# Spockuto/drand

Hardware: AMD Instinct MI355X
Metric: beacons verified/s (batch chain verify) (higher is better)
Workload: dtype u32 (381-bit Montgomery, 12x32-bit limbs); 1 GPU; configs[1]: 1000000-round chained beacon history per GPU, chain.VerifyBeacon per round; beacons_per_gpu=1000000, segment_len=64, parallelism=range-shard x1

## Files before the change

### drand_amd/_lib.py

```python
from __future__ import annotations

import ctypes
import os

_HERE = os.path.dirname(os.path.abspath(__file__))
LIB_PATH = os.environ.get("DRAND_AMD_LIB", os.path.join(_HERE, "libblsverify.so"))

BLSV_OK = 0
BLSV_EINVAL = -1
BLSV_EHIP = -2
BLSV_ENOGROUP = -3
BLSV_ENOTENOUGH = -4

AGG_OK = 0
AGG_OK_V2 = 1
AGG_V1_RECOVER_FAIL = 2
AGG_V1_INVALID = 3
AGG_V2_RECOVER_FAIL = 4

REJ_OK = 0
REJ_LENGTH = 1
REJ_FLAG = 2
REJ_INF_NONZERO = 3
REJ_X_GE_P = 4
# ... 30 lines not shown
sz = ctypes.c_size_t

SIGNATURES = {
    "blsv_version": (ctypes.c_char_p, []),
    "blsv_device_count": (ctypes.c_int, []),
    "blsv_create": (ctypes.c_int, [ctypes.c_int, ctypes.POINTER(vp)]),
    "blsv_destroy": (None, [vp]),
    "blsv_last_error": (ctypes.c_char_p, [vp]),
    "blsv_synchronize": (ctypes.c_int, [vp]),
    "blsv_set_group": (ctypes.c_int, [vp, u8p, sz, sz]),
    "blsv_verify_chained": (ctypes.c_int, [vp, ctypes.c_uint64, u8p, sz, u8p, sz, u8p, u64p, u8p]),
    "blsv_verify_chained_multi": (ctypes.c_int, [ctypes.POINTER(vp), sz, ctypes.POINTER(sz), ctypes.c_uint64, u8p, sz,
                                                  u8p, sz, u8p, u64p, u8p]),
    "blsv_verify_prevs": (ctypes.c_int, [vp, ctypes.c_uint64, u8p, sz, u8p, sz, u8p, u64p, u8p]),
    "blsv_verify_unchained": (ctypes.c_int, [vp, u64p, ctypes.c_uint64, u8p, sz, u8p, u64p, u8p]),
    "blsv_verify_messages": (ctypes.c_int, [vp, u8p, u8p, u32p, sz, u8p, u8p, u64p, u8p]),
    "blsv_verify_partials": (ctypes.c_int, [vp, u8p, sz, u8p, sz, sz, u8p, u8p]),
    "blsv_verify_partials_multi": (ctypes.c_int, [vp, u8p, u32p, u8p, sz, sz, u8p, u8p]),
    "blsv_recover": (ctypes.c_int, [vp, u8p, sz, u8p, sz, sz, sz, sz, u8p]),
    "blsv_aggregate": (ctypes.c_int, [vp, u8p, sz, u8p, sz, sz, sz, sz, u8p, u8p, u8p, u8p]),
    "blsv_aggregate_round": (ctypes.c_int, [vp, u8p, sz, u8p, sz, u8p, sz, u8p, sz, sz, sz, sz, u8p, u8p, u8p, u8p,
                                             ctypes.POINTER(ctypes.c_int32), u8p]),
    "blsv_sign": (ctypes.c_int, [vp, u8p, ctypes.c_int32, u8p, u32p, sz, u8p]),
    "blsv_verify_chained_dev": (ctypes.c_int, [vp, ctypes.c_uint64, ctypes.c_uint64, ctypes.c_uint64, vp, sz, vp, sz,
                                                vp, vp, vp, vp]),
    "blsv_generate_chained_dev": (ctypes.c_int, [vp, u8p, ctypes.c_uint64, ctypes.c_uint64, vp, sz, vp, sz, vp]),
    "blsv_profile_enable": (ctypes.c_int, [vp, ctypes.c_int]),
    "blsv_profile_read": (ctypes.c_int, [vp, ctypes.POINTER(ctypes.c_double), u64p, u64p, ctypes.c_int]),
    "blsv_lat_trace": (ctypes.c_int, [vp, u64p, ctypes.c_int, ctypes.POINTER(ctypes.c_double), ctypes.c_int]),
    "blsv_test_fp_mul": (ctypes.c_int, [vp, u32p, u32p, sz, u32p]),
    "blsv_test_op": (ctypes.c_int, [vp, ctypes.c_char_p, u32p, sz, u32p]),
    "blsv_test_op_info": (ctypes.c_int, [ctypes.c_int, ctypes.POINTER(ctypes.c_char_p), ctypes.POINTER(ctypes.c_int),
                                         ctypes.POINTER(ctypes.c_int), ctypes.POINTER(ctypes.c_int)]),
    "blsv_test_pairing": (ctypes.c_int, [vp, u32p, u32p, sz, u32p]),
    "blsv_test_hash_to_g2": (ctypes.c_int, [vp, u8p, u32p, sz, u32p, u8p]),
    "blsv_test_final_exp": (ctypes.c_int, [vp, u32p, sz, u32p, u32p]),
    "blsv_test_tail_split": (ctypes.c_int, [vp, sz]),
    "blsv_set_lat_max": (sz, [vp, sz]),
    "blsv_set_chunk": (sz, [vp, sz]),
    "blsv_workspace_bytes": (sz, [vp]),
    "blsv_lat_trace_enable": (ctypes.c_int, [vp, ctypes.c_int]),
    "blsv_test_generic_chains": (ctypes.c_int, [vp, ctypes.c_int]),
    "blsv_test_spec_stats": (ctypes.c_int, [vp, ctypes.POINTER(ctypes.c_uint64), ctypes.POINTER(ctypes.c_uint64)]),
    "blsv_test_lagrange": (ctypes.c_int, [ctypes.POINTER(ctypes.c_uint32), ctypes.c_size_t, ctypes.POINTER(ctypes.c_uint32)]),
    "blsv_service_create": (ctypes.c_int, [ctypes.c_int, ctypes.c_uint32, ctypes.c_uint32, ctypes.POINTER(vp)]),
    "blsv_service_destroy": (None, [vp]),
    "blsv_service_verify_partial": (ctypes.c_int, [vp, u8p, sz, sz, u8p, sz, u8p, sz, u8p, u8p]),
    "blsv_service_verify_recovered": (ctypes.c_int, [vp, u8p, u8p, sz, u8p, u8p, u8p]),
    "blsv_service_stats": (ctypes.c_int, [vp, u64p, u64p, u64p]),
    "blsv_test_service_limits": (ctypes.c_int, [vp, sz, sz, sz, u64p]),
    "blsv_verify_chained_rlc": (ctypes.c_int, [vp, ctypes.c_uint64, u8p, sz, u8p, sz, u8p, u64p, u8p]),
    "blsv_verify_unchained_rlc": (ctypes.c_int, [vp, u64p, ctypes.c_uint64, u8p, sz, u8p, u64p, u8p]),
    "blsv_verify_chained_rlc_dev": (ctypes.c_int, [vp, ctypes.c_uint64, ctypes.c_uint64, ctypes.c_uint64, vp, sz, vp,
                                                    sz, vp, vp, vp, vp]),
    "blsv_set_rlc_group": (sz, [vp, sz]),
    "blsv_rlc_stats": (ctypes.c_int, [vp, u64p, u64p, u64p]),
    "blsv_test_rlc_seed": (ctypes.c_int, [vp, u8p]),
    "blsv_test_rlc_sums": (ctypes.c_int, [vp, ctypes.c_uint64, u8p, sz, u8p, sz, u8p, u8p]),
    "blsv_tlock_open": (ctypes.c_int, [vp, u8p, u8p, sz, u8p, u8p, u8p, u8p]),
    "blsv_tlock_open_dev": (ctypes.c_int, [vp, u8p, vp, sz, vp, vp, vp]),
    "blsv_tlock_stats": (ctypes.c_int, [vp, u64p, u64p]),
    "blsv_tlock_open_rounds": (ctypes.c_int, [vp, u8p, u64p, sz, u8p, sz, u8p, u8p, u8p, u8p]),
    "blsv_tlock_open_rounds_dev": (ctypes.c_int, [vp, u8p, u64p, sz, vp, sz, vp, vp, vp, vp]),
    "blsv_tlock_open_rounds_stats": (ctypes.c_int, [vp, u64p, u64p]),
    "blsv_set_tlock_dense_min": (sz, [vp, sz]),
    "blsv_set_tlock_lat_max": (sz, [vp, sz]),
# ... 73 lines not shown
```

### drand_amd/csrc/fp.h

```cpp
#pragma once
#include <stdint.h>
#include "bls_constants.h"

#ifdef BLS_HOST
#include <stddef.h>
#define DI inline
#define NOINL static inline
namespace bls {
extern unsigned long long g_fp_mul_count;
}
#define BLS_COUNT_MUL() (++::bls::g_fp_mul_count)
#else
#include <hip/hip_runtime.h>
#define DI __device__ __forceinline__
#define NOINL static __device__ __noinline__
#define BLS_COUNT_MUL() ((void)0)
#endif

namespace bls {

struct fp {
  uint32_t l[12];
};

DI fp fp_load_const(const uint32_t (&c)[12]) {
  fp r;
#pragma unroll
  for (int i = 0; i < 12; i++) r.l[i] = c[i];
  return r;
}

DI fp fp_zero() {
  fp r;
#pragma unroll
  for (int i = 0; i < 12; i++) r.l[i] = 0;
  return r;
}

DI fp fp_one() { return fp_load_const(FP_ONE); }

DI bool fp_raw_is_zero(const fp& a) {
  uint32_t acc = 0;
#pragma unroll
  for (int i = 0; i < 12; i++) acc |= a.l[i];
  return acc == 0;
}

DI bool fp_is_zero(const fp& a) {
  uint32_t z = 0, q = 0;
// ... 220 lines not shown
DI u12 fp_add_raw_u12(const u12& a, const u12& b) {
  u12 r;
  unsigned c = 0;
#pragma unroll
  for (int i = 0; i < 12; i++) r[i] = __builtin_addc(a[i], b[i], c, &c);
  return r;
}

typedef uint32_t u24 __attribute__((ext_vector_type(24)));

template <bool DOT>
DI void fp_mont_dot_t(const uint32_t (&x0)[14], const uint32_t (&y0)[14], const uint32_t (&x1)[14],
                      const uint32_t (&y1)[14], uint32_t (&t)[14]) {
  uint32_t m[14];
  uint64_t c = 0;
#pragma unroll
  for (int k = 0; k < 27; k++) {
    const int lo = k > 13 ? k - 13 : 0, hi = k < 13 ? k : 13;
#pragma unroll
    for (int j = lo; j <= hi; j++) {
      c += (uint64_t)x0[j] * y0[k - j];
      if (DOT) c += (uint64_t)x1[j] * y1[k - j];
    }
    if (k < 14) {
#pragma unroll
      for (int j = 0; j < k; j++) c += (uint64_t)m[j] * P28[k - j];
      m[k] = ((uint32_t)c * P_INV28) & M28;
      c += (uint64_t)m[k] * P28[0];
    } else {
#pragma unroll
      for (int j = k - 13; j < 14; j++) c += (uint64_t)m[j] * P28[k - j];
      t[k - 14] = (uint32_t)c & M28;
    }
    c >>= 28;
  }
  t[13] = (uint32_t)c;
}
template <int NT>
DI u12 fp_mont_dot3(const uint32_t (&x0)[14], const uint32_t (&y0)[14], const uint32_t (&x1)[14],
                    const uint32_t (&y1)[14], const uint32_t (&x2)[14], const uint32_t (&y2)[14]) {
  uint32_t m[14], t[14];
  uint64_t c = 0;
#pragma unroll
  for (int k = 0; k < 27; k++) {
    const int lo = k > 13 ? k - 13 : 0, hi = k < 13 ? k : 13;
#pragma unroll
    for (int j = lo; j <= hi; j++) {
      c += (uint64_t)x0[j] * y0[k - j];
      c += (uint64_t)x1[j] * y1[k - j];
      if (NT == 3) c += (uint64_t)x2[j] * y2[k - j];
    }
    if (k < 14) {
#pragma unroll
      for (int j = 0; j < k; j++) c += (uint64_t)m[j] * P28[k - j];
      m[k] = ((uint32_t)c * P_INV28) & M28;
      c += (uint64_t)m[k] * P28[0];
    } else {
#pragma unroll
      for (int j = k - 13; j < 14; j++) c += (uint64_t)m[j] * P28[k - j];
      t[k - 14] = (uint32_t)c & M28;
    }
    c >>= 28;
  }
  t[13] = (uint32_t)c;
  return fp_join28(t);
}
// ... 108 lines not shown
  return u24_of(fp_join28(t0), fp_join28(t1));
}

template <bool KARA>
DI u24 fp2_mul_body_t(const u24& a, const u12& b0, const u12& b1) {
  if (KARA) return fp2_mul_body_kara(a, b0, b1);
  uint32_t x0[14], x1[14], y0[14], y1[14], yn[14];
  fp_split28(u24_lo(a), x0);
  fp_split28(u24_hi(a), x1);
  fp_split28(b0, y0);
  fp_split28(b1, y1);
  fp_neg28(y1, yn);
  const u12 c0 = fp_mont_dot<true>(x0, y0, x1, yn);
  BLS_SCHED_FENCE();
  const u12 c1 = fp_mont_dot<true>(x0, y1, x1, y0);
  return u24_of(c0, c1);
}
DI u24 fp2_mul_body(const u24& a, const u12& b0, const u12& b1) { return fp2_mul_body_t<BLS_FP2_KARA>(a, b0, b1); }

DI u24 fp2_sqr_body(const u24& a) {
  uint32_t s0[14], s1[14], x[14], y[14];
  fp_split28(u24_lo(a), s0);
  fp_split28(u24_hi(a), s1);
#pragma unroll
  for (int k = 0; k < 14; k++) {
    x[k] = s0[k] + s1[k];
    y[k] = s0[k] + (NEG28_16P[k] - s1[k]);
  }
  const u12 c0 = fp_mont_dot<false>(x, y, x, y);
  BLS_SCHED_FENCE();
#pragma unroll
  for (int k = 0; k < 14; k++) x[k] = s0[k] << 1;
  const u12 c1 = fp_mont_dot<false>(x, s1, x, s1);
  return u24_of(c0, c1);
}

NOINL u24 fp2_mul_u24(u24 a) {
  BLS_COUNT_MUL();
  BLS_COUNT_MUL();
  BLS_COUNT_MUL();
  const unsigned l = bls_lane();
  u12 b0, b1;
#pragma unroll
  for (int i = 0; i < 12; i++) {
    b0[i] = g_fp2_arg[i * BLS_LANES + l];
    b1[i] = g_fp2_arg[(12 + i) * BLS_LANES + l];
  }
  return fp2_mul_body(a, b0, b1);
}

NOINL u24 fp2_sqr_u24(u24 a) {
  BLS_COUNT_MUL();
  BLS_COUNT_MUL();
  return fp2_sqr_body(a);
}

DI u12 fp_to_u12(const fp& a) {
  u12 v;
#pragma unroll
  for (int i = 0; i < 12; i++) v[i] = a.l[i];
  return v;
}

DI fp fp_from_u12(const u12& v) {
  fp a;
#pragma unroll
// ... 317 lines not shown
```

### drand_amd/csrc/pairing.h

```cpp
#pragma once
#include "curve.h"

namespace bls {

struct g2proj {
  fp2 x, y, z;
};

DI fp2 fp2_mul_3b(const fp2& c) {
  fp2 x4 = fp2_dbl(fp2_dbl(fp2_mul_xi(c)));
  return fp2_add(fp2_dbl(x4), x4);
}

template <bool INL = false>
DI void miller_dbl_step(g2proj& t, fp2& l00, fp2& l01, fp2& l11, const fp& xp, const fp& yp) {
  auto mul = [](const fp2& a, const fp2& b) { return INL ? fp2_mul_inl(a, b) : fp2_mul(a, b); };
  auto sqr = [](const fp2& a) { return INL ? fp2_sqr_inl(a) : fp2_sqr(a); };
  fp2 A = fp2_half(mul(t.x, t.y));
  fp2 B = sqr(t.y);
  fp2 C = sqr(t.z);
  fp2 E = fp2_mul_3b(C);
  fp2 F = fp2_mul3(E);
  fp2 G = fp2_half(fp2_add(B, F));
  fp2 H = fp2_sub(sqr(fp2_add_lazy(t.y, t.z)), fp2_add(B, C));
  fp2 X2 = sqr(t.x);
  l00 = fp2_sub(E, B);
  l01 = fp2_mul_fp(fp2_mul3(X2), xp);
  l11 = fp2_neg(fp2_mul_fp(H, yp));
  t.x = mul(A, fp2_sub(B, F));
  t.y = fp2_sub(sqr(G), fp2_mul3(sqr(E)));
  t.z = mul(B, H);
}



struct g2proj_reg {
  g2proj& t;
  DI fp2 get(int c) const { return c == 0 ? t.x : c == 1 ? t.y : t.z; }
  DI void set(int c, const fp2& v) const {
    if (c == 0) t.x = v;
    else if (c == 1) t.y = v;
    else t.z = v;
  }
};

template <typename TS, typename Put, typename XP, typename YP>
DI void miller_dbl_step_ts(const TS& t, Put put, XP xp, YP yp) {
  const fp2 B = fp2_sqr_inl(t.get(1));
  BLS_SCHED_FENCE();
  const fp2 C = fp2_sqr_inl(t.get(2));
  BLS_SCHED_FENCE();
  const fp2 H = fp2_sub(fp2_sqr_inl(fp2_add_lazy(t.get(1), t.get(2))), fp2_add(B, C));
  BLS_SCHED_FENCE();
  put(2, fp2_neg(fp2_mul_fp_inl(H, yp())));
  BLS_SCHED_FENCE();
  t.set(2, fp2_mul_inl_k<0>(B, H));
  BLS_SCHED_FENCE();
  const fp2 E = fp2_mul_3b(C);
  const fp2 F = fp2_mul3(E);
  const fp2 G = fp2_half(fp2_add(B, F));
  put(0, fp2_sub(E, B));
  const fp2 BF = fp2_sub(B, F);
  const fp2 A = fp2_half(fp2_mul_inl_k<1>(t.get(0), t.get(1)));
  BLS_SCHED_FENCE();
  put(1, fp2_mul_fp_inl(fp2_mul3(fp2_sqr_inl(t.get(0))), xp()));
  BLS_SCHED_FENCE();
  t.set(0, fp2_mul_inl(A, BF));
  BLS_SCHED_FENCE();
  const fp2 G2 = fp2_sqr_inl(G);
  BLS_SCHED_FENCE();
  t.set(1, fp2_sub(G2, fp2_mul3(fp2_sqr_inl(E))));
}

template <typename TS, typename Put, typename Q, typename XP, typename YP>
DI void miller_add_step_ts(const TS& t, Q qload, Put put, XP xp, YP yp) {
  fp2 theta, delta;
  {
    const g2a q = qload();
    theta = fp2_sub(t.get(1), fp2_mul_inl(q.y, t.get(2)));
    BLS_SCHED_FENCE();
    delta = fp2_sub(t.get(0), fp2_mul_inl(q.x, t.get(2)));
    BLS_SCHED_FENCE();
    const fp2 u = fp2_mul_inl(theta, q.x);
    BLS_SCHED_FENCE();
    put(0, fp2_sub(u, fp2_mul_inl(delta, q.y)));
    BLS_SCHED_FENCE();
  }
  put(1, fp2_neg(fp2_mul_fp_inl(theta, xp())));
  BLS_SCHED_FENCE();
  put(2, fp2_mul_fp_inl(delta, yp()));
  BLS_SCHED_FENCE();
  const fp2 C = fp2_sqr_inl(theta);
  BLS_SCHED_FENCE();
  const fp2 D = fp2_sqr_inl(delta);
  BLS_SCHED_FENCE();
  const fp2 E = fp2_mul_inl(D, delta);
  BLS_SCHED_FENCE();
  const fp2 F = fp2_mul_inl(t.get(2), C);
  BLS_SCHED_FENCE();
  const fp2 G = fp2_mul_inl(t.get(0), D);
  BLS_SCHED_FENCE();
  const fp2 H = fp2_sub(fp2_add(E, F), fp2_dbl(G));
  t.set(0, fp2_mul_inl(delta, H));
  BLS_SCHED_FENCE();
// ... 237 lines not shown
```

### drand_amd/csrc/testhooks.cpp

```cpp
#include "../../include/blsverify_testing.h"
#include "host_internal.h"
#include "testops_list.h"

static const bls::TestOpInfo* find_test_op(const char* name, int* op) {
  if (!name) return nullptr;
  const bls::TestOpInfo* tab = bls::test_op_table();
  for (int k = 0; k < bls::TOP_COUNT; k++)
    if (!strcmp(tab[k].name, name)) {
      if (op) *op = k;
      return &tab[k];
    }
  return nullptr;
}

extern "C" {

int blsv_test_lagrange(const uint32_t* idx, size_t t, uint32_t* out) {
  if (!idx || !out) return BLSV_EINVAL;
  for (size_t i = 0; i < t; i++)
    for (size_t j = 0; j < i; j++)
      if (idx[i] == idx[j]) return BLSV_EINVAL;
  host_lagrange(idx, t, out);
  return BLSV_OK;
}

int blsv_test_rlc_seed(blsv_ctx* c, const uint8_t* seed32) {
  if (!c) return BLSV_EINVAL;
  c->rlc.seed_pinned = seed32 != nullptr;
  if (seed32) memcpy(c->rlc.seed, seed32, 32);
  return BLSV_OK;
}

int blsv_test_rlc_sums(blsv_ctx* c, uint64_t first_round, const uint8_t* prev0, size_t prev0_len,
                       const uint8_t* sigs96, size_t n, uint8_t* out_a96, uint8_t* out_b96) {
  if (!c) return BLSV_EINVAL;
  if (!n || !sigs96 || !prev0 || !out_a96 || !out_b96 || (prev0_len != 32 && prev0_len != 96))
    return fail(c, BLSV_EINVAL, "test_rlc_sums: bad arguments");
  (void)hipSetDevice(c->device);
  Tail tail;
  tail.randomized = true;
// ... 120 lines not shown
  if (n > c->cap) return fail(c, BLSV_EINVAL, "test_final_exp: more than the context chunk");
  if (!n) return BLSV_OK;
  DBuf din, dout, dref;
  HIPCHK(c, din.ensure(n * 576));
  HIPCHK(c, dout.ensure(n * 576));
  HIPCHK(c, dref.ensure(n * 576));
  const Staging w = staging(c);
  HIPCHK(c, hipMemcpyAsync(din.p, f, n * 576, hipMemcpyHostToDevice, c->stream));
  HIPCHK(c, hipMemsetAsync(w.cls, 0, n, c->stream));
  blsk::launch_test_pack_fp12(din.as<uint32_t>(), n, w.F, c->stream);
  blsk::launch_test_final_exp_ref(w.F, n, dref.as<uint32_t>(), c->stream);
  const size_t mn = tail_split_main(n, c->tail_q);
  final_exp(c, n, 0, mn, w.cls, c->stream, dout.as<uint32_t>());
  final_exp(c, n, mn, n - mn, w.cls, c->stream, dout.as<uint32_t>());
  blsk::launch_test_unpack_fp12(dout.as<uint32_t>(), n, din.as<uint32_t>(), c->stream);
  HIPCHK(c, hipMemcpyAsync(out_pipeline, din.p, n * 576, hipMemcpyDeviceToHost, c->stream));
  blsk::launch_test_unpack_fp12(dref.as<uint32_t>(), n, dout.as<uint32_t>(), c->stream);
  HIPCHK(c, hipMemcpyAsync(out_ref, dout.p, n * 576, hipMemcpyDeviceToHost, c->stream));
  HIPCHK(c, hipGetLastError());
  HIPCHK(c, hipStreamSynchronize(c->stream));
  return BLSV_OK;
}

int blsv_test_op_info(int index, const char** name, int* in_fp, int* out_fp, int* lanes) {
  if (index < 0 || index >= bls::TOP_COUNT) return BLSV_EINVAL;
  const bls::TestOpInfo& t = bls::test_op_table()[index];
  if (name) *name = t.name;
  if (in_fp) *in_fp = t.nin;
  if (out_fp) *out_fp = t.nout;
  if (lanes) *lanes = t.kind == 3 ? 3 : 1;
  return BLSV_OK;
}

int blsv_test_op(blsv_ctx* c, const char* name, const uint32_t* in, size_t n, uint32_t* out) {
  int op = 0;
  const bls::TestOpInfo* t = find_test_op(name, &op);
  if (!c || !t || (n && (!in || !out))) return BLSV_EINVAL;
  if (n > kMaxChunk) return BLSV_EINVAL;
  if (!n) return BLSV_OK;
  (void)hipSetDevice(c->device);
  const size_t in_bytes = n * (size_t)t->nin * 48, out_bytes = n * (size_t)t->nout * 48;
  DBuf din, dout, dpark;
  HIPCHK(c, din.ensure(in_bytes));
  HIPCHK(c, dout.ensure(out_bytes));
  if (t->kind == 3) HIPCHK(c, dpark.ensure(blsk::TRI_PARK_WORDS(n) * 4));
  HIPCHK(c, hipMemcpyAsync(din.p, in, in_bytes, hipMemcpyHostToDevice, c->stream));
  HIPCHK(c, hipMemsetAsync(dout.p, 0xA5, out_bytes, c->stream));
  const bool ran = t->kind == 2
                       ? blsk::launch_test_op_mf(op, din.as<uint32_t>(), n, dout.as<uint32_t>(), c->stream)
                       : blsk::launch_test_op(op, din.as<uint32_t>(), n, dout.as<uint32_t>(),
                                              t->kind == 3 ? dpark.as<uint32_t>() : nullptr, c->stream);
  if (!ran) return fail(c, BLSV_EINVAL, "test_op: no kernel for this op");
  HIPCHK(c, hipGetLastError());
  HIPCHK(c, hipMemcpyAsync(out, dout.p, out_bytes, hipMemcpyDeviceToHost, c->stream));
  HIPCHK(c, hipStreamSynchronize(c->stream));
  return BLSV_OK;
}

int blsv_test_hash_to_g2(blsv_ctx* c, const uint8_t* msgs, const uint32_t* msg_lens, size_t n, uint32_t* out,
                         uint8_t* inf) {
  if (!c || (n && (!msg_lens || !out || !inf))) return BLSV_EINVAL;
  if (n > kMaxChunk) return BLSV_EINVAL;
  (void)hipSetDevice(c->device);
  int rc = ensure_workspace(c, n);
  if (rc) return rc;
  if (n > c->cap) return fail(c, BLSV_EINVAL, "test_hash_to_g2: more than the context chunk");
// ... 15 lines not shown
```

### drand_amd/csrc/testops.h

```cpp
#pragma once
#include "pairing.h"
#include "tri.h"
#include "testops_list.h"

namespace bls {

DI fp2 t_f2(const fp* x, int k) { return {x[k], x[k + 1]}; }
DI fp6 t_f6(const fp* x, int k) { return {t_f2(x, k), t_f2(x, k + 2), t_f2(x, k + 4)}; }
DI fp12 t_f12(const fp* x, int k) { return {t_f6(x, k), t_f6(x, k + 6)}; }
DI void t_put2(fp* r, int k, const fp2& v) { r[k] = v.c0, r[k + 1] = v.c1; }
DI void t_put6(fp* r, int k, const fp6& v) { t_put2(r, k, v.c0), t_put2(r, k + 2, v.c1), t_put2(r, k + 4, v.c2); }
DI void t_put12(fp* r, int k, const fp12& v) { t_put6(r, k, v.c0), t_put6(r, k + 6, v.c1); }
DI fp t_flag(bool b) {
  fp r = fp_zero();
  r.l[0] = b ? 1u : 0u;
  return r;
}

template <int OP, typename KP16>
DI void test_op_run(const fp* x, fp* r) {
  if constexpr (OP == TOP_fp_mul) r[0] = fp_mul(x[0], x[1]);
  if constexpr (OP == TOP_fp_mul_inl) r[0] = fp_mul_inl(x[0], x[1]);
  if constexpr (OP == TOP_fp_sqr) r[0] = fp_sqr(x[0]);
  if constexpr (OP == TOP_fp_add) r[0] = fp_add(x[0], x[1]);
// ... 28 lines not shown
  if constexpr (OP == TOP_fp2_sqr) t_put2(r, 0, fp2_sqr(t_f2(x, 0)));
  if constexpr (OP == TOP_fp2_sqr_inl) t_put2(r, 0, fp2_sqr_inl(t_f2(x, 0)));
  if constexpr (OP == TOP_fp2_mul_xi) t_put2(r, 0, fp2_mul_xi(t_f2(x, 0)));
  if constexpr (OP == TOP_fp2_neg) t_put2(r, 0, fp2_neg(t_f2(x, 0)));
  if constexpr (OP == TOP_fp2_inv) t_put2(r, 0, fp2_inv(t_f2(x, 0)));
  if constexpr (OP == TOP_fp2_3u_p_2x) t_put2(r, 0, fp2_3u_pm_2x(t_f2(x, 0), t_f2(x, 2), false));
  if constexpr (OP == TOP_fp2_3u_m_2x) t_put2(r, 0, fp2_3u_pm_2x(t_f2(x, 0), t_f2(x, 2), true));
  if constexpr (OP == TOP_kara6_c0) t_put2(r, 0, kara6_c0(t_f2(x, 0), t_f2(x, 2), t_f2(x, 4), t_f2(x, 6), KP16()));
  if constexpr (OP == TOP_kara6_c1) t_put2(r, 0, kara6_c1(t_f2(x, 0), t_f2(x, 2), t_f2(x, 4), t_f2(x, 6), KP16()));
  if constexpr (OP == TOP_kara6_c2) t_put2(r, 0, kara6_c2(t_f2(x, 0), t_f2(x, 2), t_f2(x, 4), t_f2(x, 6), KP16()));
  if constexpr (OP == TOP_fp6_mul_lin) t_put6(r, 0, fp6_mul_lin(t_f6(x, 0), t_f6(x, 6), KP16()));
  if constexpr (OP == TOP_fp6_mul) t_put6(r, 0, fp6_mul(t_f6(x, 0), t_f6(x, 6)));
  if constexpr (OP == TOP_fp6_sqr) t_put6(r, 0, fp6_sqr(t_f6(x, 0)));
  if constexpr (OP == TOP_fp6_mul_by_01) t_put6(r, 0, fp6_mul_by_01(t_f6(x, 0), t_f2(x, 6), t_f2(x, 8)));
  if constexpr (OP == TOP_fp6_mul_by_1) t_put6(r, 0, fp6_mul_by_1(t_f6(x, 0), t_f2(x, 6)));
  if constexpr (OP == TOP_fp6_mul_by_12) t_put6(r, 0, fp6_mul_by_12(t_f6(x, 0), t_f2(x, 6), t_f2(x, 8)));
  if constexpr (OP == TOP_fp6_inv) t_put6(r, 0, fp6_inv(t_f6(x, 0)));
  if constexpr (OP == TOP_fp4_sqr_k7) {
    const fp4 y = fp4_sqr_k7(fp4{t_f2(x, 0), t_f2(x, 2)});
    t_put2(r, 0, y.a), t_put2(r, 2, y.b);
  }
  if constexpr (OP == TOP_fp12_mul) t_put12(r, 0, fp12_mul(t_f12(x, 0), t_f12(x, 12)));
  if constexpr (OP == TOP_fp12_sqr) t_put12(r, 0, fp12_sqr(t_f12(x, 0)));
  if constexpr (OP == TOP_fp12_sqr_lin) t_put12(r, 0, fp12_sqr_lin(t_f12(x, 0), KP16()));
  if constexpr (OP == TOP_fp12_mul_by_014)
    t_put12(r, 0, fp12_mul_by_014(t_f12(x, 0), t_f2(x, 12), t_f2(x, 14), t_f2(x, 16)));
  if constexpr (OP == TOP_line_mul_line)
    t_put12(r, 0, line_mul_line(line{t_f2(x, 0), t_f2(x, 2), t_f2(x, 4)}, line{t_f2(x, 6), t_f2(x, 8), t_f2(x, 10)}));
  if constexpr (OP == TOP_fp12_cyclotomic_sqr) t_put12(r, 0, fp12_cyclotomic_sqr(t_f12(x, 0)));
  if constexpr (OP == TOP_fp12_frob) t_put12(r, 0, fp12_frob(t_f12(x, 0)));
  if constexpr (OP == TOP_fp12_frob2) t_put12(r, 0, fp12_frob2(t_f12(x, 0)));
  if constexpr (OP == TOP_fp12_conj) t_put12(r, 0, fp12_conj(t_f12(x, 0)));
  if constexpr (OP == TOP_fp12_inv) t_put12(r, 0, fp12_inv(t_f12(x, 0)));
}

}
```

### drand_amd/csrc/testops_list.h

```cpp
#pragma once

#define BLS_TEST_OPS(X)                                                                              \
  X(fp_mul, 2, 1, 0) X(fp_mul_inl, 2, 1, 0) X(fp_sqr, 1, 1, 0) X(fp_add, 2, 1, 0) X(fp_sub, 2, 1, 0) \
  X(fp_addsub_add, 2, 1, 0) X(fp_addsub_sub, 2, 1, 0) X(fp_neg, 1, 1, 0) X(fp_half, 1, 1, 0)         \
  X(fp_dbl, 1, 1, 0) X(fp_mul3, 1, 1, 0) X(fp_add_lazy_mul, 3, 2, 0) X(fp_add_lazy2_mul, 5, 2, 0)   \
  X(fp_canon, 1, 1, 0) X(fp_is_zero, 1, 1, 0) X(fp_eq, 2, 1, 0) X(fp_inv_bingcd_raw, 1, 2, 0)        \
  X(fp_inv, 1, 1, 0) X(fp_pow_sqrt_inv, 1, 1, 0)                                                     \
  X(fp2_mul, 4, 2, 0) X(fp2_mul_inl, 4, 2, 0) X(fp2_mul_inl_kara, 4, 2, 0) X(fp2_sqr, 2, 2, 0)       \
  X(fp2_sqr_inl, 2, 2, 0) X(fp2_mul_xi, 2, 2, 0) X(fp2_neg, 2, 2, 0) X(fp2_inv, 2, 2, 0)             \
  X(fp2_3u_p_2x, 4, 2, 0) X(fp2_3u_m_2x, 4, 2, 0) X(fp2_3u_p_2x_lds, 4, 2, 1)                        \
  X(fp2_3u_m_2x_lds, 4, 2, 1) X(kara6_c0, 8, 2, 0) X(kara6_c1, 8, 2, 0) X(kara6_c2, 8, 2, 0)         \
  X(fp6_mul_lin, 12, 6, 0) X(fp6_mul, 12, 6, 0) X(fp6_sqr, 6, 6, 0) X(fp6_mul_by_01, 10, 6, 0)       \
  X(fp6_mul_by_1, 8, 6, 0) X(fp6_mul_by_12, 10, 6, 0) X(fp6_inv, 6, 6, 0) X(fp4_sqr_k7, 4, 4, 0)     \
  X(fp4_sqr_dot, 4, 4, 1) X(fp4_mul, 8, 4, 1) X(fp12_mul, 24, 12, 0) X(fp12_sqr, 12, 12, 0)          \
  X(fp12_sqr_lin, 12, 12, 0) X(fp12_mul_by_014, 18, 12, 0) X(line_mul_line, 12, 12, 0)               \
  X(fp12_cyclotomic_sqr, 12, 12, 0) X(fp12_frob, 12, 12, 0) X(fp12_frob2, 12, 12, 0)                 \
  X(fp12_conj, 12, 12, 0) X(fp12_inv, 12, 12, 0)                                                     \
  X(fp6_mul_lb, 12, 6, 2) X(fp12_mul_by_line_pair_lds, 22, 12, 2)                                    \
  X(tri_cyclotomic_sqr, 12, 12, 3) X(tri_mul_lp, 24, 12, 3) X(tri_sqr_lp, 12, 12, 3)                 \
  X(tri_line_pair, 12, 12, 3) X(tri_frob, 12, 12, 3) X(tri_frob2, 12, 12, 3) X(tri_conj, 12, 12, 3)  \
  X(tri_is_one, 12, 1, 3)

namespace bls {

enum TestOp : int {
#define X(name, nin, nout, kind) TOP_##name,
  BLS_TEST_OPS(X)
#undef X
      TOP_COUNT
};

struct TestOpInfo {
  const char* name;
  int nin, nout, kind;
};
inline const TestOpInfo* test_op_table() {
  static const TestOpInfo tab[TOP_COUNT] = {
#define X(name, nin, nout, kind) {#name, nin, nout, kind},
      BLS_TEST_OPS(X)
#undef X
  };
  return tab;
}

}
```

### drand_amd/csrc/tower.h

```cpp
#pragma once
#include "fp.h"

namespace bls {

struct fp2 {
  fp c0, c1;
};
struct fp6 {
  fp2 c0, c1, c2;
};
struct fp12 {
  fp6 c0, c1;
};

DI fp2 fp2_load_const(const uint32_t (&c)[2][12]) { return {fp_load_const(c[0]), fp_load_const(c[1])}; }
DI fp2 fp2_zero() { return {fp_zero(), fp_zero()}; }
DI fp2 fp2_one() { return {fp_one(), fp_zero()}; }
DI bool fp2_is_zero(const fp2& a) { return fp_is_zero(a.c0) & fp_is_zero(a.c1); }
DI bool fp2_eq(const fp2& a, const fp2& b) { return fp_eq(a.c0, b.c0) & fp_eq(a.c1, b.c1); }
DI fp2 fp2_select(bool c, const fp2& a, const fp2& b) { return {fp_select(c, a.c0, b.c0), fp_select(c, a.c1, b.c1)}; }
DI fp2 fp2_add(const fp2& a, const fp2& b) {
  uint32_t s0[12], d0[12], s1[12], d1[12];
  unsigned c0 = 0, b0 = 0, c1 = 0, b1 = 0;
#pragma unroll
// ... 150 lines not shown
  for (int i = 0; i < 12; i++) {
    r.c0.l[i] = d0[i] & m0;
    r.c1.l[i] = d1[i] & m1;
  }
  return r;
}
DI fp2 fp2_conj(const fp2& a) { return {a.c0, fp_neg(a.c1)}; }

DI u24 fp2_to_u24(const fp2& a) { return u24_of(fp_to_u12(a.c0), fp_to_u12(a.c1)); }
DI fp2 fp2_from_u24(const u24& v) { return {fp_from_u12(u24_lo(v)), fp_from_u12(u24_hi(v))}; }

DI fp2 fp2_mul(const fp2& a, const fp2& b) {
  fp2_arg_store(fp2_to_u24(b));
  return fp2_from_u24(fp2_mul_u24(fp2_to_u24(a)));
}
DI fp2 fp2_sqr(const fp2& a) { return fp2_from_u24(fp2_sqr_u24(fp2_to_u24(a))); }
template <bool KARA>
DI fp2 fp2_mul_inl_t(const fp2& a, const fp2& b) {
  BLS_COUNT_MUL();
  BLS_COUNT_MUL();
  BLS_COUNT_MUL();
  return fp2_from_u24(fp2_mul_body_t<KARA>(fp2_to_u24(a), fp_to_u12(b.c0), fp_to_u12(b.c1)));
}
DI fp2 fp2_mul_inl(const fp2& a, const fp2& b) { return fp2_mul_inl_t<BLS_FP2_KARA_INL>(a, b); }
#ifndef BLS_LINES_KARA
#define BLS_LINES_KARA 3
#endif
template <int SITE>
DI fp2 fp2_mul_inl_k(const fp2& a, const fp2& b) { return fp2_mul_inl_t<((BLS_LINES_KARA >> SITE) & 1) != 0>(a, b); }
DI fp2 fp2_sqr_inl(const fp2& a) {
  BLS_COUNT_MUL();
  BLS_COUNT_MUL();
  return fp2_from_u24(fp2_sqr_body(fp2_to_u24(a)));
}

DI fp2 fp2_mul_fp(const fp2& a, const fp& b) { return {fp_mul(a.c0, b), fp_mul(a.c1, b)}; }
DI fp2 fp2_mul_fp_inl(const fp2& a, const fp& b) {
  const fp c0 = fp_mul_inl(a.c0, b);
  BLS_SCHED_FENCE();
  return {c0, fp_mul_inl(a.c1, b)};
}
DI fp2 fp2_mul3(const fp2& a) { return {fp_mul3(a.c0), fp_mul3(a.c1)}; }

DI fp2 fp2_mul_xi(const fp2& a) {
  uint32_t d[12], e[12], s[12], u[12];
  unsigned bd = 0, ce = 0, cs = 0, bu = 0;
#pragma unroll
  for (int i = 0; i < 12; i++) {
    d[i] = __builtin_subc(a.c0.l[i], a.c1.l[i], bd, &bd);
    s[i] = __builtin_addc(a.c0.l[i], a.c1.l[i], cs, &cs);
    e[i] = __builtin_addc(d[i], P2_RAW[i], ce, &ce);
    u[i] = __builtin_subc(s[i], P2_RAW[i], bu, &bu);
  }
  fp2 r;
#pragma unroll
  for (int i = 0; i < 12; i++) {
    r.c0.l[i] = bd ? e[i] : d[i];
    r.c1.l[i] = bu ? s[i] : u[i];
  }
  return r;
}

DI fp2 fp2_inv(const fp2& a) {
  fp n = fp_add(fp_sqr(a.c0), fp_sqr(a.c1));
  fp ni = fp_inv(n);
  return {fp_mul(a.c0, ni), fp_neg(fp_mul(a.c1, ni))};
// ... 374 lines not shown
```

### drand_amd/engine.py

```python
from __future__ import annotations

import ctypes
from dataclasses import dataclass

from . import _lib
from ._lib import u8p, u32p, u64p


class EngineError(RuntimeError):
    def __init__(self, code, msg):
        super().__init__(f"blsverify error {code}: {msg}")
        self.code = code


@dataclass
class BatchResult:
    ok: list
    first_bad: int | None
    reject_class: list

    @property
    def all_ok(self):
        return self.first_bad is None

# ... 759 lines not shown
                 "final_exp", "pow1_start", "pow1_end", "xmd_done", "sswu_done", "iso_add_done", "cofactor_done",
                 "sig_sqrt_done", "sig_subgroup_done")

    def lat_trace_enable(self, on=True):
        self._check(self.lib.blsv_lat_trace_enable(self._h, 1 if on else 0))

    def lat_trace(self, clear=True):
        n = len(self.LAT_MARKS)
        t = (ctypes.c_uint64 * n)()
        rate = ctypes.c_double()
        got = self.lib.blsv_lat_trace(self._h, t, n, ctypes.byref(rate), 1 if clear else 0)
        if got < 0:
            raise EngineError(got, self.lib.blsv_last_error(self._h).decode())
        t0 = t[0]
        return {k: (t[i] - t0) / rate.value for i, k in enumerate(self.LAT_MARKS[:got]) if t[i] and t0}

    def set_lat_max(self, n):
        return self.lib.blsv_set_lat_max(self._h, int(n))

    def set_chunk(self, items):
        return self.lib.blsv_set_chunk(self._h, int(items))

    def workspace_bytes(self):
        return self.lib.blsv_workspace_bytes(self._h)

    def test_fp_mul(self, a_limbs, b_limbs):
        n = len(a_limbs) // 12
        A = (ctypes.c_uint32 * max(len(a_limbs), 1))(*a_limbs)
        B = (ctypes.c_uint32 * max(len(b_limbs), 1))(*b_limbs)
        O = (ctypes.c_uint32 * max(n * 12, 1))()
        self._check(self.lib.blsv_test_fp_mul(self._h, A, B, n, O))
        return list(O)[:n * 12]

    def test_ops(self):
        ops, k = {}, 0
        name, a, b, c = ctypes.c_char_p(), ctypes.c_int(), ctypes.c_int(), ctypes.c_int()
        while self.lib.blsv_test_op_info(k, ctypes.byref(name), ctypes.byref(a), ctypes.byref(b), ctypes.byref(c)) == 0:
            ops[name.value.decode()] = (a.value, b.value, c.value)
            k += 1
        return ops

    def test_op(self, name, operands):
        if self._ops is None:
            self._ops = self.test_ops()
        nin, nout, _ = self._ops[name]
        if len(operands) % nin:
            raise ValueError(f"{name} takes {nin} Fp elements per item")
        n = len(operands) // nin
        raw = b"".join(int(v).to_bytes(48, "little") for v in operands)
        A = (ctypes.c_uint32 * max(len(raw) // 4, 1)).from_buffer_copy(raw if raw else bytes(4))
        O = (ctypes.c_uint32 * max(n * nout * 12, 1))()
        self._check(self.lib.blsv_test_op(self._h, name.encode(), A, n, O))
        ob = bytes(O)
        return [int.from_bytes(ob[48 * k:48 * k + 48], "little") for k in range(n * nout)]

    def test_pairing(self, p_words, q_words):
        n = len(p_words) // 24
        Pp = (ctypes.c_uint32 * max(len(p_words), 1))(*p_words)
        Q = (ctypes.c_uint32 * max(len(q_words), 1))(*q_words)
        O = (ctypes.c_uint32 * max(n * 144, 1))()
        self._check(self.lib.blsv_test_pairing(self._h, Pp, Q, n, O))
        return list(O)[:n * 144]

    def test_final_exp(self, f_words):
        n = len(f_words) // 144
        Fw = (ctypes.c_uint32 * max(len(f_words), 1))(*f_words)
        A = (ctypes.c_uint32 * max(n * 144, 1))()
        B = (ctypes.c_uint32 * max(n * 144, 1))()
        self._check(self.lib.blsv_test_final_exp(self._h, Fw, n, A, B))
        return list(A)[:n * 144], list(B)[:n * 144]

    def test_tail_split(self, q):
        self._check(self.lib.blsv_test_tail_split(self._h, ctypes.c_size_t(-1).value if q is None else int(q)))

    def test_hash_to_g2(self, msgs):
        n = len(msgs)
        lens = (ctypes.c_uint32 * max(n, 1))(*[len(m) for m in msgs])
# ... 118 lines not shown
```

### include/blsverify_testing.h

```cpp
#ifndef DRAND_AMD_BLSVERIFY_TESTING_H
#define DRAND_AMD_BLSVERIFY_TESTING_H

#include "blsverify.h"

#ifdef __cplusplus
extern "C" {
#endif

int blsv_test_fp_mul(blsv_ctx* ctx, const uint32_t* a, const uint32_t* b, size_t n, uint32_t* out);

int blsv_test_pairing(blsv_ctx* ctx, const uint32_t* p, const uint32_t* q, size_t n, uint32_t* out_f);

int blsv_test_final_exp(blsv_ctx* ctx, const uint32_t* f, size_t n, uint32_t* out_pipeline, uint32_t* out_ref);

int blsv_test_tail_split(blsv_ctx* ctx, size_t q);

int blsv_test_tauth_walk_waves(blsv_ctx* ctx, int waves);

int blsv_test_op(blsv_ctx* ctx, const char* name, const uint32_t* in, size_t n, uint32_t* out);
int blsv_test_op_info(int index, const char** name, int* in_fp, int* out_fp, int* lanes);

int blsv_test_hash_to_g2(blsv_ctx* ctx, const uint8_t* msgs, const uint32_t* msg_lens, size_t n, uint32_t* out,
                         uint8_t* inf);

int blsv_test_generic_chains(blsv_ctx* ctx, int on);

int blsv_test_spec_stats(blsv_ctx* ctx, uint64_t* hits, uint64_t* misses);

int blsv_test_service_limits(blsv_service* svc, size_t chunk, size_t lat_max, size_t arena_entries,
                             uint64_t* sub_launches);

int blsv_profile_enable(blsv_ctx* ctx, int on);
int blsv_lat_trace(blsv_ctx* ctx, uint64_t* ticks, int n, double* ticks_per_us, int clear);
int blsv_lat_trace_enable(blsv_ctx* ctx, int on);
int blsv_profile_read(blsv_ctx* ctx, double* ms, uint64_t* launches, uint64_t* items, int nstages);
int blsv_test_lagrange(const uint32_t* idx, size_t t, uint32_t* out);

int blsv_test_rlc_seed(blsv_ctx* ctx, const uint8_t* seed32);
int blsv_test_rlc_sums(blsv_ctx* ctx, uint64_t first_round, const uint8_t* prev0, size_t prev0_len,
                       const uint8_t* sigs96, size_t n, uint8_t* out_a96, uint8_t* out_b96);

#ifdef __cplusplus
}
#endif

#endif
```

Baseline: 2.512 million beacons/s.

## Fuse G²−E·F in Miller doubling and derive XY from squares

```diff
diff --git a/drand_amd/_lib.py b/drand_amd/_lib.py
--- a/drand_amd/_lib.py
+++ b/drand_amd/_lib.py
@@ -86,6 +86,9 @@
     "blsv_test_op": (ctypes.c_int, [vp, ctypes.c_char_p, u32p, sz, u32p]),
     "blsv_test_op_info": (ctypes.c_int, [ctypes.c_int, ctypes.POINTER(ctypes.c_char_p), ctypes.POINTER(ctypes.c_int),
                                          ctypes.POINTER(ctypes.c_int), ctypes.POINTER(ctypes.c_int)]),
+    "blsv_test_step_op_info": (ctypes.c_int, [ctypes.c_int, ctypes.POINTER(ctypes.c_char_p),
+                                              ctypes.POINTER(ctypes.c_int), ctypes.POINTER(ctypes.c_int),
+                                              ctypes.POINTER(ctypes.c_int)]),
     "blsv_test_pairing": (ctypes.c_int, [vp, u32p, u32p, sz, u32p]),
     "blsv_test_hash_to_g2": (ctypes.c_int, [vp, u8p, u32p, sz, u32p, u8p]),
     "blsv_test_final_exp": (ctypes.c_int, [vp, u32p, sz, u32p, u32p]),
diff --git a/drand_amd/csrc/fp.h b/drand_amd/csrc/fp.h
--- a/drand_amd/csrc/fp.h
+++ b/drand_amd/csrc/fp.h
@@ -10,11 +10,20 @@
 extern unsigned long long g_fp_mul_count;
 }
 #define BLS_COUNT_MUL() (++::bls::g_fp_mul_count)
+#ifdef BLS_HOST_COLUMNS
+namespace bls {
+extern unsigned long long g_col_max;
+}
+#define BLS_COLUMN(c) (::bls::g_col_max = (c) > ::bls::g_col_max ? (c) : ::bls::g_col_max)
+#else
+#define BLS_COLUMN(c) ((void)0)
+#endif
 #else
 #include <hip/hip_runtime.h>
 #define DI __device__ __forceinline__
 #define NOINL static __device__ __noinline__
 #define BLS_COUNT_MUL() ((void)0)
+#define BLS_COLUMN(c) ((void)0)
 #endif
 
 namespace bls {
@@ -301,6 +310,7 @@
       for (int j = k - 13; j < 14; j++) c += (uint64_t)m[j] * P28[k - j];
       t[k - 14] = (uint32_t)c & M28;
     }
+    BLS_COLUMN(c);
     c >>= 28;
   }
   t[13] = (uint32_t)c;
@@ -475,6 +485,36 @@
 #pragma unroll
   for (int k = 0; k < 14; k++) x[k] = s0[k] << 1;
   const u12 c1 = fp_mont_dot<false>(x, s1, x, s1);
+  return u24_of(c0, c1);
+}
+
+DI u24 fp2_sqr_minus_prod_body(const u24& g, const u24& e, const u24& f) {
+  uint32_t g0[14], g1[14], e1[14], f0[14], x0[14], y0[14], x1[14], y1[14];
+  fp_split28(u24_lo(g), g0);
+  fp_split28(u24_hi(g), g1);
+  fp_split28(u24_hi(e), e1);
+  fp_split28(u24_lo(f), f0);
+  {
+    uint32_t e0[14], f1[14];
+    fp_split28(u24_lo(e), e0);
+    fp_split28(u24_hi(f), f1);
+#pragma unroll
+    for (int k = 0; k < 14; k++) {
+      x0[k] = g0[k] + g1[k];
+      y0[k] = g0[k] + (NEG28_16P[k] - g1[k]);
+      x1[k] = f0[k] + f1[k];
+      y1[k] = e1[k] + (NEG28_16P[k] - e0[k]);
+    }
+  }
+  const u12 c0 = fp_mont_dot<true>(x0, y0, x1, y1);
+  BLS_SCHED_FENCE();
+#pragma unroll
+  for (int k = 0; k < 14; k++) {
+    x0[k] = g0[k] << 1;
+    x1[k] = f0[k] << 1;
+    y1[k] = NEG28_16P[k] - e1[k];
+  }
+  const u12 c1 = fp_mont_dot<true>(x0, g1, x1, y1);
   return u24_of(c0, c1);
 }
 
diff --git a/drand_amd/csrc/pairing.h b/drand_amd/csrc/pairing.h
--- a/drand_amd/csrc/pairing.h
+++ b/drand_amd/csrc/pairing.h
@@ -44,6 +44,13 @@
   }
 };
 
+#ifndef BLS_LINES_XY_SQR
+#define BLS_LINES_XY_SQR 1
+#endif
+DI fp2 miller_dbl_xy_open(const fp2& X, const fp2& Y, const fp2& B) {
+  return fp2_sub(fp2_sqr_inl(fp2_add_lazy(X, Y)), B);
+}
+DI fp2 miller_dbl_xy_close(const fp2& S, const fp2& X2) { return fp2_half(fp2_half(fp2_sub(S, X2))); }
 template <typename TS, typename Put, typename XP, typename YP>
 DI void miller_dbl_step_ts(const TS& t, Put put, XP xp, YP yp) {
   const fp2 B = fp2_sqr_inl(t.get(1));
@@ -55,21 +62,28 @@
   put(2, fp2_neg(fp2_mul_fp_inl(H, yp())));
   BLS_SCHED_FENCE();
   t.set(2, fp2_mul_inl_k<0>(B, H));
+  BLS_SCHED_FENCE();
+#if BLS_LINES_XY_SQR
+  fp2 A = miller_dbl_xy_open(t.get(0), t.get(1), B);
+#else
+  fp2 A = fp2_half(fp2_mul_inl_k<1>(t.get(0), t.get(1)));
+#endif
   BLS_SCHED_FENCE();
   const fp2 E = fp2_mul_3b(C);
   const fp2 F = fp2_mul3(E);
   const fp2 G = fp2_half(fp2_add(B, F));
   put(0, fp2_sub(E, B));
   const fp2 BF = fp2_sub(B, F);
-  const fp2 A = fp2_half(fp2_mul_inl_k<1>(t.get(0), t.get(1)));
-  BLS_SCHED_FENCE();
-  put(1, fp2_mul_fp_inl(fp2_mul3(fp2_sqr_inl(t.get(0))), xp()));
+  t.set(1, fp2_sqr_minus_prod_inl(G, E, F));
+  BLS_SCHED_FENCE();
+  const fp2 X2 = fp2_sqr_inl(t.get(0));
+#if BLS_LINES_XY_SQR
+  A = miller_dbl_xy_close(A, X2);
+#endif
+  BLS_SCHED_FENCE();
+  put(1, fp2_mul_fp_inl(fp2_mul3(X2), xp()));
   BLS_SCHED_FENCE();
   t.set(0, fp2_mul_inl(A, BF));
-  BLS_SCHED_FENCE();
-  const fp2 G2 = fp2_sqr_inl(G);
-  BLS_SCHED_FENCE();
-  t.set(1, fp2_sub(G2, fp2_mul3(fp2_sqr_inl(E))));
 }
 
 template <typename TS, typename Put, typename Q, typename XP, typename YP>
diff --git a/drand_amd/csrc/testhooks.cpp b/drand_amd/csrc/testhooks.cpp
--- a/drand_amd/csrc/testhooks.cpp
+++ b/drand_amd/csrc/testhooks.cpp
@@ -5,7 +5,7 @@
 static const bls::TestOpInfo* find_test_op(const char* name, int* op) {
   if (!name) return nullptr;
   const bls::TestOpInfo* tab = bls::test_op_table();
-  for (int k = 0; k < bls::TOP_COUNT; k++)
+  for (int k = 0; k < bls::TOP_ALL; k++)
     if (!strcmp(tab[k].name, name)) {
       if (op) *op = k;
       return &tab[k];
@@ -192,6 +192,16 @@
   return BLSV_OK;
 }
 
+int blsv_test_step_op_info(int index, const char** name, int* in_fp, int* out_fp, int* lanes) {
+  if (index < 0 || index >= bls::TOP_ALL - bls::TOP_COUNT) return BLSV_EINVAL;
+  const bls::TestOpInfo& t = bls::test_op_table()[bls::TOP_COUNT + index];
+  if (name) *name = t.name;
+  if (in_fp) *in_fp = t.nin;
+  if (out_fp) *out_fp = t.nout;
+  if (lanes) *lanes = t.kind == 3 ? 3 : 1;
+  return BLSV_OK;
+}
+
 int blsv_test_op(blsv_ctx* c, const char* name, const uint32_t* in, size_t n, uint32_t* out) {
   int op = 0;
   const bls::TestOpInfo* t = find_test_op(name, &op);
diff --git a/drand_amd/csrc/testops.h b/drand_amd/csrc/testops.h
--- a/drand_amd/csrc/testops.h
+++ b/drand_amd/csrc/testops.h
@@ -84,6 +84,19 @@
   if constexpr (OP == TOP_fp12_frob2) t_put12(r, 0, fp12_frob2(t_f12(x, 0)));
   if constexpr (OP == TOP_fp12_conj) t_put12(r, 0, fp12_conj(t_f12(x, 0)));
   if constexpr (OP == TOP_fp12_inv) t_put12(r, 0, fp12_inv(t_f12(x, 0)));
+  if constexpr (OP == TOP_fp2_sqr_minus_prod_inl)
+    t_put2(r, 0, fp2_sqr_minus_prod_inl(t_f2(x, 0), t_f2(x, 2), t_f2(x, 4)));
+  if constexpr (OP == TOP_miller_dbl_xy_half) {
+    const fp2 X = t_f2(x, 0), Y = t_f2(x, 2);
+    t_put2(r, 0, miller_dbl_xy_close(miller_dbl_xy_open(X, Y, fp2_sqr_inl(Y)), fp2_sqr_inl(X)));
+  }
+  if constexpr (OP == TOP_miller_dbl_step_ts) {
+    g2proj T = {t_f2(x, 0), t_f2(x, 2), t_f2(x, 4)};
+    miller_dbl_step_ts(
+        g2proj_reg{T}, [&](int c, const fp2& v) { t_put2(r, 6 + 2 * c, v); }, [&]() { return x[6]; },
+        [&]() { return x[7]; });
+    t_put2(r, 0, T.x), t_put2(r, 2, T.y), t_put2(r, 4, T.z);
+  }
 }
 
 }
diff --git a/drand_amd/csrc/testops_list.h b/drand_amd/csrc/testops_list.h
--- a/drand_amd/csrc/testops_list.h
+++ b/drand_amd/csrc/testops_list.h
@@ -21,13 +21,21 @@
   X(tri_line_pair, 12, 12, 3) X(tri_frob, 12, 12, 3) X(tri_frob2, 12, 12, 3) X(tri_conj, 12, 12, 3)  \
   X(tri_is_one, 12, 1, 3)
 
+#define BLS_TEST_STEP_OPS(X) \
+  X(fp2_sqr_minus_prod_inl, 6, 2, 0) X(miller_dbl_xy_half, 4, 2, 0) X(miller_dbl_step_ts, 8, 12, 0)
+
 namespace bls {
 
 enum TestOp : int {
 #define X(name, nin, nout, kind) TOP_##name,
   BLS_TEST_OPS(X)
 #undef X
-      TOP_COUNT
+      TOP_COUNT,
+  TOP_STEP_BASE = TOP_COUNT - 1,
+#define X(name, nin, nout, kind) TOP_##name,
+  BLS_TEST_STEP_OPS(X)
+#undef X
+      TOP_ALL
 };
 
 struct TestOpInfo {
@@ -35,9 +43,9 @@
   int nin, nout, kind;
 };
 inline const TestOpInfo* test_op_table() {
-  static const TestOpInfo tab[TOP_COUNT] = {
+  static const TestOpInfo tab[TOP_ALL] = {
 #define X(name, nin, nout, kind) {#name, nin, nout, kind},
-      BLS_TEST_OPS(X)
+      BLS_TEST_OPS(X) BLS_TEST_STEP_OPS(X)
 #undef X
   };
   return tab;
diff --git a/drand_amd/csrc/tower.h b/drand_amd/csrc/tower.h
--- a/drand_amd/csrc/tower.h
+++ b/drand_amd/csrc/tower.h
@@ -206,6 +206,13 @@
   BLS_COUNT_MUL();
   BLS_COUNT_MUL();
   return fp2_from_u24(fp2_sqr_body(fp2_to_u24(a)));
+}
+DI fp2 fp2_sqr_minus_prod_inl(const fp2& g, const fp2& e, const fp2& f) {
+  BLS_COUNT_MUL();
+  BLS_COUNT_MUL();
+  BLS_COUNT_MUL();
+  BLS_COUNT_MUL();
+  return fp2_from_u24(fp2_sqr_minus_prod_body(fp2_to_u24(g), fp2_to_u24(e), fp2_to_u24(f)));
 }
 
 DI fp2 fp2_mul_fp(const fp2& a, const fp& b) { return {fp_mul(a.c0, b), fp_mul(a.c1, b)}; }
diff --git a/drand_amd/engine.py b/drand_amd/engine.py
--- a/drand_amd/engine.py
+++ b/drand_amd/engine.py
@@ -815,17 +815,23 @@
         self._check(self.lib.blsv_test_fp_mul(self._h, A, B, n, O))
         return list(O)[:n * 12]
 
-    def test_ops(self):
+    def _enum_ops(self, info):
         ops, k = {}, 0
         name, a, b, c = ctypes.c_char_p(), ctypes.c_int(), ctypes.c_int(), ctypes.c_int()
-        while self.lib.blsv_test_op_info(k, ctypes.byref(name), ctypes.byref(a), ctypes.byref(b), ctypes.byref(c)) == 0:
+        while info(k, ctypes.byref(name), ctypes.byref(a), ctypes.byref(b), ctypes.byref(c)) == 0:
             ops[name.value.decode()] = (a.value, b.value, c.value)
             k += 1
         return ops
 
+    def test_ops(self):
+        return self._enum_ops(self.lib.blsv_test_op_info)
+
+    def test_step_ops(self):
+        return self._enum_ops(self.lib.blsv_test_step_op_info)
+
     def test_op(self, name, operands):
         if self._ops is None:
-            self._ops = self.test_ops()
+            self._ops = {**self.test_ops(), **self.test_step_ops()}
         nin, nout, _ = self._ops[name]
         if len(operands) % nin:
             raise ValueError(f"{name} takes {nin} Fp elements per item")
diff --git a/include/blsverify_testing.h b/include/blsverify_testing.h
--- a/include/blsverify_testing.h
+++ b/include/blsverify_testing.h
@@ -19,6 +19,7 @@
 
 int blsv_test_op(blsv_ctx* ctx, const char* name, const uint32_t* in, size_t n, uint32_t* out);
 int blsv_test_op_info(int index, const char** name, int* in_fp, int* out_fp, int* lanes);
+int blsv_test_step_op_info(int index, const char** name, int* in_fp, int* out_fp, int* lanes);
 
 int blsv_test_hash_to_g2(blsv_ctx* ctx, const uint8_t* msgs, const uint32_t* msg_lens, size_t n, uint32_t* out,
                          uint8_t* inf);
```

Result: no change. 2.529 million beacons/s, median of 6 (+0.7%).
